# GoatWu/AdaLog

Hardware: NVIDIA B200
Metric: fpcs_candidates_per_s (higher is better)
Workload: dtype int8 + bf16 operands holding exact integers (s32 / f32 accumulate), f64 error sums

## Files before the change

### adalog_b200/_lib.py

```python
import ctypes
import os

_HERE = os.path.dirname(os.path.abspath(__file__))
LIB_PATH = os.path.join(_HERE, 'csrc', 'libadalog_b200.so')

c_f32p = ctypes.c_void_p
c_i64 = ctypes.c_int64
c_int = ctypes.c_int
c_vp = ctypes.c_void_p


class GemmErrArgs(ctypes.Structure):
    _fields_ = [
        ('A', c_vp), ('Bm', c_vp), ('a_rows', c_i64), ('b_rows', c_i64),
        ('KB', ctypes.c_int32), ('N', ctypes.c_int32), ('BN', ctypes.c_int32), ('U', ctypes.c_int32),
        ('UG', ctypes.c_int32), ('upc', ctypes.c_int32), ('S', ctypes.c_int32), ('dtype', ctypes.c_int32),
        ('order', ctypes.c_int32), ('reserved', ctypes.c_int32),
        ('brpg', c_i64), ('g_base', c_i64), ('u_base', c_i64),
        ('y', c_vp), ('ldy', c_i64),
        ('rs', c_vp), ('rb', c_vp), ('rs_div', c_i64), ('rs_mod', c_i64),
        ('cs', c_vp), ('cb', c_vp),
        ('partial', c_vp),
    ]

# ... 32 lines not shown
    'adalog_uniform_fakequant_f32': [c_vp, c_vp, c_vp, c_i64, c_vp, c_vp, c_i64, c_i64, c_int, c_int, c_vp],
    'adalog_log_fakequant_f32': [c_vp, c_vp, c_vp, c_i64, c_vp, c_int, c_int, c_vp, c_vp, c_vp, c_vp, c_int, c_vp],
    'adalog_twin_fakequant_f32': [c_vp, c_vp, c_i64, c_vp, c_int, c_vp],
    'adalog_sweep_err_w_self': [c_vp, c_int, c_int, c_vp, c_vp, c_int, c_int, c_vp, c_vp],
    'adalog_sweep_err_a_self': [c_vp, c_i64, c_int, c_int, c_vp, c_vp, c_int, c_int, c_vp, c_int, c_vp],
    'adalog_gen_uniform_fixed': [c_vp, c_i64, c_int, c_i64, c_vp, c_vp, c_i64, c_i64, c_int, c_vp, c_int, c_vp, c_int, c_vp],
    'adalog_gen_uniform_cand': [c_vp, c_i64, c_int, c_i64, c_vp, c_vp, c_int, c_i64, c_i64, c_i64, c_i64, c_i64, c_int,
                                c_vp, c_int, c_int, c_vp, c_int, c_vp],
    'adalog_gen_log_cand': [c_vp, c_i64, c_int, c_i64, c_vp, c_vp, c_int, c_vp, c_vp, c_int, c_vp, c_int, c_vp],
    'adalog_gen_log_fixed': [c_vp, c_i64, c_int, c_i64, c_vp, c_vp, c_vp, c_vp, c_vp, c_int, c_vp, c_int, c_vp],
    'adalog_gen_split3': [c_vp, c_i64, c_int, c_i64, c_vp, c_int, c_vp],
    'adalog_select_init': [c_vp, c_i64, c_int, c_vp, c_vp],
    'adalog_select_hist': [c_vp, c_i64, c_i64, c_i64, c_vp, c_i64, c_i64, c_int, c_int, c_int, c_vp],
    'adalog_select_scan': [c_vp, c_i64, c_int, c_int, c_vp],
    'adalog_select_finish': [c_vp, c_i64, c_int, c_vp, c_vp],
    'adalog_cand_gemm_err_grid': [ctypes.POINTER(GemmErrArgs)],
    'adalog_cand_gemm_err': [ctypes.POINTER(GemmErrArgs), c_vp],
    'adalog_fused_cand_gemm_err_grid': [ctypes.POINTER(FusedArgs)],
    'adalog_fused_cand_gemm_err': [ctypes.POINTER(FusedArgs), c_vp],
    'adalog_lin_fused_cand_gemm_err_grid': [ctypes.POINTER(LinFusedArgs)],
    'adalog_lin_fused_cand_gemm_err_passes': [ctypes.POINTER(LinFusedArgs)],
    'adalog_lin_fused_cand_gemm_err': [ctypes.POINTER(LinFusedArgs), c_vp],
    'adalog_gemm_dequant': [ctypes.POINTER(GemmErrArgs), c_vp, c_i64, c_i64, c_vp],
    'adalog_debug_gemm_tile': [c_vp, c_vp, c_int, c_int, c_vp, c_vp, c_vp, c_vp, c_int, c_vp],
}

OTHER_SYMBOLS = {'adalog_last_error', 'adalog_select_workspace_bytes', 'adalog_select_hist_ptr'}

_lib = None
LAUNCHES = {'count': 0}
_NO_LAUNCH = {'adalog_version', 'adalog_cand_gemm_err_grid', 'adalog_fused_cand_gemm_err_grid',
              'adalog_lin_fused_cand_gemm_err_grid', 'adalog_lin_fused_cand_gemm_err_passes'}


class AdalogError(RuntimeError):
    pass


def load():
    global _lib
    if _lib is not None:
        return _lib
    if not os.path.exists(LIB_PATH):
        raise AdalogError(f'{LIB_PATH} not found: build it with `python __graft_entry__.py` '
                          f'(adalog_b200 has no CPU fallback)')
    lib = ctypes.CDLL(LIB_PATH)
# ... 23 lines not shown
```

### adalog_b200/csrc/gemm_err.cu

```cuda
#include "common.cuh"
#include "tc_common.cuh"
#include "../../include/adalog_b200.h"
#include <cuda.h>
#include <cudaTypedefs.h>
#include <stdlib.h>
#include <type_traits>

namespace adalog {

constexpr int kMaxBN = 256;
constexpr int kStages = 4;
constexpr int kAccStages = 2;
constexpr uint32_t kABytes = kBM * kBK * 2;
constexpr uint32_t kBBytes = kMaxBN * kBK * 2;
constexpr uint32_t kTmemCols = 512;
constexpr int kEpiWarp0 = 0;
constexpr int kEpiWarps = 8;
constexpr int kEpiGroups = kEpiWarps / 4;
constexpr int kEpiThreads = kEpiWarps * 32;
constexpr int kTmaWarp = kEpiWarps, kMmaWarp = kEpiWarps + 1;
constexpr int kThreads = (kMmaWarp + 1) * 32;

constexpr int kCsCols = 1024;
constexpr int kSlabsPerGroup = (kMaxBN / 32 + kEpiGroups - 1) / kEpiGroups;
struct __align__(16) SmemTail {
  float ysw[kEpiWarps][kSlabsPerGroup * 32];
  float cs_all[kCsCols + kMaxBN];
  float cb_all[kCsCols + kMaxBN];
  uint64_t full[kStages];
  uint64_t empty[kStages];
  uint64_t tfull[kAccStages];
  uint64_t tempty[kAccStages];
  uint32_t tmem_base;
  uint32_t pad;
  double comb[kEpiGroups - 1][kBM];
};
constexpr size_t kSmemBytes = 1024  + (size_t)kStages * (kABytes + kBBytes);

struct KArgs {
  int KB, N, BN, NT, U, UG, upc, cpg;
  int gx, S, split_fast;
  long long brpg, g_base, u_base;
  const float* y; long long ldy;
  const float* rs; const float* rb; long long rs_div, rs_mod;
  const float* cs; const float* cb;
  double* partial;
  float* dbg;
  float* out; long long ldo; long long m_rows;
};

enum { MODE_CS = 0, MODE_RB = 1, MODE_PLAIN = 2, MODE_NOEPI = 3 ,
       MODE_STORE = 4 };

template <int MODE, bool DEBUG, bool I8>
__global__ void __maxnreg__(152)
cand_gemm_err_kernel(const __grid_constant__ CUtensorMap tmA, const __grid_constant__ CUtensorMap tmB, const KArgs a) {
  extern __shared__ uint8_t smem_raw[];
  uint8_t* smem = reinterpret_cast<uint8_t*>((reinterpret_cast<uintptr_t>(smem_raw) + 1023) & ~(uintptr_t)1023);
  uint8_t* sA = smem;
  uint8_t* sB = smem + (size_t)kStages * kABytes;
  __shared__ SmemTail tail_s;
  SmemTail* tail = &tail_s;

  const int warp = uniform_warp_idx();
  const int lane = threadIdx.x & 31;

  const int bx = a.split_fast ? (int)(blockIdx.x / a.S) : (int)(blockIdx.x % a.gx);
  const int by = a.split_fast ? (int)(blockIdx.x % a.S) : (int)(blockIdx.x / a.gx);
  const int g_local = bx / a.cpg;
  const int ci = bx - g_local * a.cpg;
  const int u0 = g_local * a.UG + (int)(((long long)ci * a.UG) / a.cpg);
  const int u1 = min(g_local * a.UG + (int)(((long long)(ci + 1) * a.UG) / a.cpg), a.U);
  const int nt0 = (int)(((long long)by * a.NT) / a.S);
  const int nt1 = (int)(((long long)(by + 1) * a.NT) / a.S);
  const int n_units = max(u1 - u0, 0);
// ... 38 lines not shown
    }
  } else if (warp == kMmaWarp) {
    {
      uint32_t stage = 0, phase = 0;
      const uint32_t idesc = I8 ? make_idesc_i8(a.BN) : make_idesc(a.BN);
      const uint32_t sA_u = smem_u32(sA), sB_u = smem_u32(sB);
      for (int t = 0; t < n_tiles; ++t) {
        const uint32_t as = t & 1, aphase = (t >> 1) & 1;
        mbar_wait(&tail->tempty[as], aphase ^ 1);
        tc_fence_after();
        const uint32_t tmem_d = tmem_base + as * kMaxBN;
        for (int kb = 0; kb < a.KB; ++kb) {
          mbar_wait(&tail->full[stage], phase);
          tc_fence_after();
          umma_kblock_commit<I8>(tmem_d, make_smem_desc(sA_u + stage * kABytes), make_smem_desc(sB_u + stage * kBBytes),
                                 idesc, kb != 0 ? 1u : 0u, 4, smem_u32(&tail->empty[stage]));
          if (++stage == kStages) { stage = 0; phase ^= 1; }
        }
        umma_commit_elect(smem_u32(&tail->tfull[as]));
      }
    }
  } else if (warp < kTmaWarp) {
    constexpr bool HAS_CS = MODE == MODE_CS || MODE == MODE_STORE;
    constexpr bool STORE = MODE == MODE_STORE;
    const int ew = warp - kEpiWarp0;
    const int eg = ew >> 2;
    const int et = ((warp & 3) << 5) | lane;
    const uint32_t lane_base = (uint32_t)((warp & 3) * 32) << 16;
    constexpr int G = kEpiGroups;
    float* const ysw = tail_s.ysw[ew];
    TwoSumF acc;
    float rs = 0.0f, rb = 0.0f;
    long long cur_ri = -1;
    float yreg[kSlabsPerGroup];
#pragma unroll
    for (int i = 0; i < kSlabsPerGroup; ++i) yreg[i] = 0.0f;
    if (HAS_CS) {
      const int st = threadIdx.x - kEpiWarp0 * 32;
      const int ncs = n_nt * a.BN;
      for (int idx = st; idx < kCsCols + kMaxBN; idx += kEpiThreads) {
        float cv = 0.0f, bv = 0.0f;
        if (idx < ncs) {
          const int ti = idx / a.BN;
          const int c = idx - ti * a.BN;
          const int n = (nt0 + ti) * a.BN + c;
          if (n < a.N) { cv = __ldg(a.cs + n); bv = __ldg(a.cb + n); }
        }
        tail_s.cs_all[idx] = cv;
        tail_s.cb_all[idx] = bv;
      }
      asm volatile("bar.sync 1, %0;" ::"n"(kEpiThreads) : "memory");
    }
    auto prefetch = [&](int u, int n0) {
#pragma unroll
      for (int i = 0; i < kSlabsPerGroup; ++i) {
        const int c = (eg + i * G) * 32 + lane;
        const int n = n0 + c;
        yreg[i] = (!STORE && c < a.BN && n < a.N) ? __ldg(a.y + (long long)u * a.ldy + n) : 0.0f;
      }
    };
    float acc4[4];
    auto accf = [](uint32_t w) -> float { return I8 ? __int2float_rn((int)w) : __uint_as_float(w); };
    float* orow = nullptr;
    int ocol = 0;
    const bool ovec = STORE && (a.ldo & 3) == 0 && (reinterpret_cast<uintptr_t>(a.out) & 15) == 0;
    auto quad = [&](auto masked, const uint32_t (&d)[32], int j, int l0, int cc, int lim, float rs, float rb) {
      constexpr bool MASKED = decltype(masked)::value;
      const float4 yv = *reinterpret_cast<const float4*>(&ysw[l0 + j]);
      const float y4[4] = {yv.x, yv.y, yv.z, yv.w};
      float c4[4] = {1.0f, 1.0f, 1.0f, 1.0f};
      if (HAS_CS) {
        const float4 cv = *reinterpret_cast<const float4*>(&tail_s.cs_all[cc + j]);
        c4[0] = cv.x; c4[1] = cv.y; c4[2] = cv.z; c4[3] = cv.w;
      }
      if (STORE) {
        const float4 bv = *reinterpret_cast<const float4*>(&tail_s.cb_all[cc + j]);
        float4 o;
        o.x = fmaf(rs * c4[0], accf(d[j + 0]), bv.x); o.y = fmaf(rs * c4[1], accf(d[j + 1]), bv.y);
        o.z = fmaf(rs * c4[2], accf(d[j + 2]), bv.z); o.w = fmaf(rs * c4[3], accf(d[j + 3]), bv.w);
        if (orow != nullptr) {
          float* dst = orow + ocol + j;
          if (!MASKED || j + 3 < lim) {
            if (ovec) *reinterpret_cast<float4*>(dst) = o;
            else { dst[0] = o.x; dst[1] = o.y; dst[2] = o.z; dst[3] = o.w; }
          } else {
            if (j + 0 < lim) dst[0] = o.x;
            if (j + 1 < lim) dst[1] = o.y;
            if (j + 2 < lim) dst[2] = o.z;
          }
        }
        return;
      }
      if (!MASKED) {
        const float f0 = accf(d[j]), f1 = accf(d[j + 1]), f2 = accf(d[j + 2]), f3 = accf(d[j + 3]);
        float e0, e1, e2, e3;
        if (HAS_CS) {
          float t0, t1, t2, t3;
          fmul2(t0, t1, f0, f1, c4[0], c4[1]);
          fmul2(t2, t3, f2, f3, c4[2], c4[3]);
          ffma2(e0, e1, -rs, -rs, t0, t1, y4[0], y4[1]);
          ffma2(e2, e3, -rs, -rs, t2, t3, y4[2], y4[3]);
        } else if (MODE == MODE_RB) {
// ... 7 lines not shown
          ffma2(e2, e3, -rs, -rs, f2, f3, y4[2], y4[3]);
        }
        ffma2(acc4[0], acc4[1], e0, e1, e0, e1, acc4[0], acc4[1]);
        ffma2(acc4[2], acc4[3], e2, e3, e2, e3, acc4[2], acc4[3]);
        return;
      }
#pragma unroll
      for (int e = 0; e < 4; ++e) {
        float diff;
        if (HAS_CS) diff = fmaf(-rs, accf(d[j + e]) * c4[e], y4[e]);
        else if (MODE == MODE_RB) diff = y4[e] - fmaf(rs, accf(d[j + e]), rb);
        else diff = fmaf(-rs, accf(d[j + e]), y4[e]);
        diff = (j + e < lim) ? diff : 0.0f;
        acc4[e] = fmaf(diff, diff, acc4[e]);
      }
    };
    auto consume = [&](const uint32_t (&d)[32], int c0, int l0, int cc, int lim, float rs, float rb, int n0, int ncols) {
      if (DEBUG) {
#pragma unroll
        for (int j = 0; j < 32; ++j)
          if (c0 + j < ncols) a.dbg[(long long)et * a.N + n0 + c0 + j] = accf(d[j]);
      }
      ocol = c0;
      if (MODE == MODE_NOEPI) {
        acc4[0] += __uint_as_float(d[0]);
      } else if (lim >= 32) {
#pragma unroll
        for (int j = 0; j < 32; j += 4) quad(std::false_type{}, d, j, l0, cc, 32, rs, rb);
      } else {
#pragma unroll
        for (int j = 0; j < 32; j += 4)
          if (j < lim) quad(std::true_type{}, d, j, l0, cc, lim, rs, rb);
      }
    };
    int cu = u0, cnt = 0;
    long long ri = 0, rrem = 0;
    if (n_tiles > 0) {
      const long long gu = a.u_base + cu;
      ri = (gu / a.rs_div) % a.rs_mod;
      rrem = gu % a.rs_div;
      prefetch(cu, (nt0 + cnt) * a.BN);
    }
    for (int t = 0; t < n_tiles; ++t) {
      const int n0 = (nt0 + cnt) * a.BN;
      const int toff = cnt * a.BN;
      const int ncols = min(a.BN, a.N - n0);
      const long long ri_t = ri;
      if (STORE) {
        const long long row = (a.u_base + cu) * kBM + et;
        orow = row < a.m_rows ? a.out + row * a.ldo + n0 : nullptr;
      }
      if (++cnt == n_nt) {
        cnt = 0; ++cu;
        if (++rrem == a.rs_div) { rrem = 0; if (++ri == a.rs_mod) ri = 0; }
      }
      const uint32_t as = t & 1, aphase = (t >> 1) & 1;
      __syncwarp();
#pragma unroll
      for (int i = 0; i < kSlabsPerGroup; ++i)
        ysw[i * 32 + lane] = HAS_CS ? yreg[i] - tail_s.cb_all[toff + (eg + i * G) * 32 + lane] : yreg[i];
      __syncwarp();
      if (t + 1 < n_tiles) prefetch(cu, (nt0 + cnt) * a.BN);
      if (ri_t != cur_ri) {
        cur_ri = ri_t;
        rs = __ldg(a.rs + ri_t * kBM + et);
        rb = (MODE == MODE_RB) ? __ldg(a.rb + ri_t * kBM + et) : 0.0f;
      }
      mbar_wait(&tail->tfull[as], aphase);
      tc_fence_after();
      acc4[0] = acc4[1] = acc4[2] = acc4[3] = 0.0f;
      const uint32_t tbase = tmem_base + lane_base + as * kMaxBN;
      const int nslab = (ncols + 31) >> 5;
      uint32_t da[32], db[32];
      if (eg < nslab) tmem_ld32(tbase + eg * 32, da);
      int l0 = 0;
      constexpr bool SLAB64 = MODE == MODE_RB;
      auto flush = [&]() {
        acc.add((acc4[0] + acc4[1]) + (acc4[2] + acc4[3]));
        acc4[0] = acc4[1] = acc4[2] = acc4[3] = 0.0f;
      };
      for (int sl = eg; sl < nslab; sl += 2 * G, l0 += 64) {
        tmem_ld_wait();
        if (sl + G < nslab) tmem_ld32(tbase + (sl + G) * 32, db);
        consume(da, sl * 32, l0, toff + sl * 32, ncols - sl * 32, rs, rb, n0, ncols);
        if (SLAB64) flush();
        if (sl + G < nslab) {
          tmem_ld_wait();
          if (sl + 2 * G < nslab) tmem_ld32(tbase + (sl + 2 * G) * 32, da);
          consume(db, (sl + G) * 32, l0 + 32, toff + (sl + G) * 32, ncols - (sl + G) * 32, rs, rb, n0, ncols);
          if (SLAB64) flush();
        }
      }
      if (!SLAB64) acc.add((acc4[0] + acc4[1]) + (acc4[2] + acc4[3]));
      tc_fence_before();
      __syncwarp();
      if (lane == 0) mbar_arrive(&tail->tempty[as]);
    }
    const double acc64 = acc.value();
    if (eg > 0) tail_s.comb[eg - 1][et] = acc64;
    asm volatile("bar.sync 1, %0;" ::"n"(kEpiThreads) : "memory");
    if (eg == 0 && a.partial) {
      double tot = acc64;
#pragma unroll
      for (int g = 1; g < kEpiGroups; ++g) tot += tail_s.comb[g - 1][et];
      a.partial[((long long)by * a.gx + bx) * kBM + et] = tot;
    }
  }

  tc_fence_before();
  __syncthreads();
  if (warp == kMmaWarp) {
    __syncwarp();
    tc_fence_after();
    asm volatile("tcgen05.dealloc.cta_group::1.sync.aligned.b32 %0, %1;" ::"r"(tmem_base), "r"(kTmemCols) : "memory");
  }
}

static int validate(const adalog_gemm_err_args* a, bool need_partial) {
  ADALOG_REQUIRE(a && a->A && a->Bm, -1, "cand_gemm_err: null operand");
  ADALOG_REQUIRE(a->KB > 0 && a->N > 0 && a->U > 0 && a->UG > 0 && a->upc > 0 && a->S > 0, -1,
                 "cand_gemm_err: non-positive size");
  ADALOG_REQUIRE(a->BN >= 16 && a->BN <= kMaxBN && a->BN % 16 == 0, -1, "cand_gemm_err: BN must be a multiple of 16 in [16,256]");
  ADALOG_REQUIRE(a->dtype == ADALOG_BF16 || a->dtype == ADALOG_I8, -1, "cand_gemm_err: dtype must be ADALOG_BF16 or ADALOG_I8");
  ADALOG_REQUIRE(a->order == ADALOG_ORDER_UNIT_FAST || a->order == ADALOG_ORDER_SPLIT_FAST, -1, "cand_gemm_err: bad order");
  ADALOG_REQUIRE(a->U % a->UG == 0, -1, "cand_gemm_err: U must be a multiple of UG");
  ADALOG_REQUIRE(a->a_rows >= (int64_t)a->U * kBM, -1, "cand_gemm_err: A has fewer than U*128 rows");
  ADALOG_REQUIRE(a->rs_div > 0 && a->rs_mod > 0 && a->rs, -1, "cand_gemm_err: row scale required");
  ADALOG_REQUIRE((a->cs == nullptr) == (a->cb == nullptr), -1, "cand_gemm_err: cs and cb come together");
  ADALOG_REQUIRE(!a->rb || a->cs || a->BN % 32 == 0, -1,
                 "cand_gemm_err: with a row bias (W-side sweeps) BN must be a multiple of 32 (per-slab FP64 promotion)");
  ADALOG_REQUIRE(a->y && (a->partial || !need_partial), -1, "cand_gemm_err: y / partial required");
  const int NT = (a->N + a->BN - 1) / a->BN;
  ADALOG_REQUIRE(a->S <= NT, -1, "cand_gemm_err: more N splits than N tiles");
  ADALOG_REQUIRE(!a->cs || ((NT + a->S - 1) / a->S) * a->BN <= kCsCols, -1,
                 "cand_gemm_err: with column scales a CTA covers at most 1024 columns (raise S)");
  return 0;
}

static int launch(const adalog_gemm_err_args* a, float* dbg, cudaStream_t st, float* out = nullptr, long long ldo = 0,
                  long long m_rows = 0) {
  KArgs k;
  k.out = out; k.ldo = ldo; k.m_rows = m_rows;
  k.KB = a->KB; k.N = a->N; k.BN = a->BN; k.NT = (a->N + a->BN - 1) / a->BN; k.U = a->U; k.UG = a->UG; k.upc = a->upc;
  k.cpg = (a->UG + a->upc - 1) / a->upc;
  k.brpg = a->brpg; k.g_base = a->g_base; k.u_base = a->u_base;
  k.y = a->y; k.ldy = a->ldy; k.rs = a->rs; k.rb = a->rb; k.rs_div = a->rs_div; k.rs_mod = a->rs_mod;
  k.cs = a->cs; k.cb = a->cb; k.partial = a->partial; k.dbg = dbg;
  CUtensorMap tmA, tmB;
  const bool i8 = a->dtype == ADALOG_I8;
  const int64_t cols = (int64_t)a->KB * (i8 ? 2 * kBK : kBK);
  int rc = make_map(&tmA, a->A, a->a_rows, cols, kBM, i8);
  if (rc) return rc;
  rc = make_map(&tmB, a->Bm, a->b_rows, cols, a->BN, i8);
  if (rc) return rc;
  k.gx = (a->U / a->UG) * k.cpg; k.S = a->S; k.split_fast = a->order == ADALOG_ORDER_SPLIT_FAST;
  dim3 grid((unsigned)((long long)k.gx * k.S));
#define ADALOG_LAUNCH_GEMM(MD, DBG, I8)                                                                       \
  do {                                                                                                        \
    cudaFuncSetAttribute(cand_gemm_err_kernel<MD, DBG, I8>, cudaFuncAttributeMaxDynamicSharedMemorySize,      \
                         (int)kSmemBytes);                                                                    \
    cand_gemm_err_kernel<MD, DBG, I8><<<grid, kThreads, kSmemBytes, st>>>(tmA, tmB, k);                       \
  } while (0)
  if (out) {
    if (i8) ADALOG_LAUNCH_GEMM(MODE_STORE, false, true);
    else    ADALOG_LAUNCH_GEMM(MODE_STORE, false, false);
  } else if (i8) {
    if (dbg)         ADALOG_LAUNCH_GEMM(MODE_PLAIN, true, true);
    else if (a->cs)  ADALOG_LAUNCH_GEMM(MODE_CS, false, true);
    else if (a->rb)  ADALOG_LAUNCH_GEMM(MODE_RB, false, true);
    else             ADALOG_LAUNCH_GEMM(MODE_PLAIN, false, true);
  } else {
    if (dbg)         ADALOG_LAUNCH_GEMM(MODE_PLAIN, true, false);
    else if (a->cs)  ADALOG_LAUNCH_GEMM(MODE_CS, false, false);
    else if (a->rb)  ADALOG_LAUNCH_GEMM(MODE_RB, false, false);
    else if (getenv("ADALOG_B200_DIAG_NOEPI")) ADALOG_LAUNCH_GEMM(MODE_NOEPI, false, false);
    else             ADALOG_LAUNCH_GEMM(MODE_PLAIN, false, false);
  }
#undef ADALOG_LAUNCH_GEMM
  return check_launch("cand_gemm_err");
}

}

using namespace adalog;

extern "C" {
// ... 1 lines not shown
int adalog_cand_gemm_err_grid(const adalog_gemm_err_args* a) {
  int rc = validate(a, false);
  if (rc) return rc;
  return (a->U / a->UG) * ((a->UG + a->upc - 1) / a->upc);
}

int adalog_cand_gemm_err(const adalog_gemm_err_args* a, void* stream) {
  int rc = validate(a, true);
  if (rc) return rc;
  return launch(a, nullptr, (cudaStream_t)stream);
}

int adalog_gemm_dequant(const adalog_gemm_err_args* a, float* out, int64_t ldo, int64_t m_rows, void* stream) {
  ADALOG_REQUIRE(a && out && m_rows > 0 && ldo >= a->N, -1, "gemm_dequant: bad output");
  ADALOG_REQUIRE(a->A && a->Bm && a->rs && a->cs && a->cb && a->KB > 0 && a->N > 0 && a->U > 0 && a->UG == a->U &&
                     a->upc > 0 && a->S > 0 && (int64_t)a->U * kBM >= m_rows && a->rs_div > 0 && a->rs_mod > 0, -1,
                 "gemm_dequant: bad arguments (one group, U = ceil(m_rows / 128), rs / cs / cb required)");
  ADALOG_REQUIRE(a->BN >= 16 && a->BN <= kMaxBN && a->BN % 16 == 0, -1, "gemm_dequant: BN must be a multiple of 16 in [16,256]");
  ADALOG_REQUIRE(a->dtype == ADALOG_BF16 || a->dtype == ADALOG_I8, -1, "gemm_dequant: dtype");
  ADALOG_REQUIRE(a->order == ADALOG_ORDER_UNIT_FAST || a->order == ADALOG_ORDER_SPLIT_FAST, -1, "gemm_dequant: order");
  const int NT = (a->N + a->BN - 1) / a->BN;
  ADALOG_REQUIRE(a->S <= NT && ((NT + a->S - 1) / a->S) * a->BN <= kCsCols, -1,
                 "gemm_dequant: a CTA covers at most 1024 columns (raise S)");
  return launch(a, nullptr, (cudaStream_t)stream, out, ldo, m_rows);
}

int adalog_debug_gemm_tile(const void* A, const void* Bm, int KB, int N, float* D, const float* zeros, const float* ones,
                           double* partial, int dtype, void* stream) {
  ADALOG_REQUIRE(A && Bm && D && zeros && ones && partial && KB > 0 && N > 0, -1, "debug_gemm_tile: bad arguments");
  double* part = partial;
  adalog_gemm_err_args a;
  memset(&a, 0, sizeof(a));
  a.A = A; a.Bm = Bm; a.a_rows = kBM; a.b_rows = N; a.KB = KB; a.N = N; a.dtype = dtype;
  a.BN = N >= kMaxBN ? kMaxBN : ((N + 15) / 16) * 16;
  a.U = 1; a.UG = 1; a.upc = 1; a.S = 1; a.brpg = N; a.g_base = 0; a.u_base = 0;
  a.y = zeros; a.ldy = 0; a.rs = ones; a.rb = nullptr; a.rs_div = 1; a.rs_mod = 1; a.cs = nullptr; a.cb = nullptr;
  a.partial = part;
  int rc = validate(&a, true);
  if (rc) return rc;
  return launch(&a, D, (cudaStream_t)stream);
}

}
```

### adalog_b200/ops.py

```python
import ctypes
import math
import threading

import torch

from . import _lib
from ._lib import AdalogError, FusedArgs, GemmErrArgs, LinFusedArgs
from ._lib import call as _lib_call

P_TILE = 128
BK = 64

PROFILE = {'on': False, 'gemm': [], 'fused': [], 'lin': []}


def profile_reset(on):
    PROFILE['on'] = bool(on)
    PROFILE['gemm'] = []
    PROFILE['fused'] = []
    PROFILE['lin'] = []


def profile_gemm_summary(split=False):
    torch.cuda.synchronize()
# ... 286 lines not shown
    else:
        call('adalog_cand_gemm_err', ctypes.byref(a), _stream())
    return partial


def gemm_dequant(A, m_rows, Bm, ka, N, rs, cs, cb, upc, S, i8=False, split_fast=False, out=None):
    _cuda(A, Bm, rs, cs, cb)
    BN = pick_bn(N)
    U = (m_rows + P_TILE - 1) // P_TILE
    a = GemmErrArgs()
    a.A, a.Bm = A.data_ptr(), Bm.data_ptr()
    a.a_rows, a.b_rows = int(m_rows), int(Bm.shape[0])
    a.KB = ka // (2 * BK if i8 else BK)
    a.dtype = I8 if i8 else BF16
    a.order = 1 if split_fast else 0
    a.N, a.BN, a.U, a.UG, a.upc, a.S = int(N), int(BN), int(U), int(U), int(upc), int(S)
    a.brpg, a.g_base, a.u_base = 0, 0, 0
    a.rs, a.rs_div, a.rs_mod = rs.data_ptr(), 1 << 62, 1
    a.cs, a.cb = cs.data_ptr(), cb.data_ptr()
    if out is None:
        out = torch.empty(m_rows, N, dtype=torch.float32, device=A.device)
    call('adalog_gemm_dequant', ctypes.byref(a), _p(out), int(out.stride(0)), int(m_rows), _stream())
    return out


SMEM_LIMIT = 227 * 1024 - 16384


def fused_plan(K, N, i8, log, n_levels):
    el = 2 * BK if i8 else BK
    KB = (K + el - 1) // el
    if N > 256 or KB > 4:
        return None
    BN = pick_bn(N)
    smem = 1024 + KB * 16384 + KB * BN * 128 + (P_TILE * (2 * n_levels + 1) * 4 if log else 0)
    if smem > SMEM_LIMIT or (log and (i8 or 2 * n_levels > 64)):
        return None
    return KB, BN


def fused_cand_gemm_err(x2d, K, Bm, N, U, UG, brpg, y, ldy, rs, rs_div, rs_mod, upc, n_levels, P, cs=None, cz=None,
                        pstride=0, gstride=0, g_div=1, g_mod=1, cq=None, mtab=None, i8=False):
    log = cq is not None
    KB, BN = fused_plan(K, N, i8, log, n_levels)
    _cuda(x2d, Bm, y, rs)
    assert x2d.dtype == torch.float32 and x2d.stride(1) == 1
# ... 102 lines not shown
```

### adalog_b200/sweep.py

```python
import functools
import math
import os

import torch

from . import _const, ops
from .quantizers._ste import flag as _flag
from .utils import dist as adist

WS_BYTES = int(os.environ.get('ADALOG_B200_WS_MB', '8192')) << 20
NUM_SMS = 148
R_BASE = 37.0
USE_I8 = os.environ.get('ADALOG_B200_I8', '1') == '1'

LIN_FUSED = os.environ.get('ADALOG_B200_LIN_FUSED', '1') != '0'


def _lin_fused_passes():
    mode = os.environ.get('ADALOG_B200_LIN_FUSED', '1')
    if not LIN_FUSED or mode == '0':
        return None
    return 1 << 30 if mode == 'force' else 1

_workspaces = {}
# ... 49 lines not shown
    if NT > 1 and unit_bytes * min(NUM_SMS, nu) > L2_CAND_BYTES:
        split_fast = True
        s_min = min(NT, max(s_min, math.ceil(unit_bytes * NUM_SMS / L2_CAND_TARGET)))
    best = None
    for S in range(s_min, min(NT, max(s_min, 16)) + 1):
        tps = math.ceil(NT / S)
        cands = {ug, 1}
        for w in range(1, 9):
            c = (NUM_SMS * w) // (groups * S)
            if c >= 1:
                cands.add(math.ceil(ug / min(c, ug)))
        for upc in cands:
            cpg = math.ceil(ug / upc)
            ctas = groups * cpg * S
            cost = math.ceil(ctas / NUM_SMS) * (math.ceil(ug / cpg) * tps * tile_cost + CTA_FIXED_COST)
            key = (cost, ctas)
            if best is None or key < best[0]:
                best = (key, upc, cpg, S)
    _, upc, cpg, S = best
    return groups, upc, cpg, S, split_fast


def run_cand_gemm(gen_cand, U, ka, UG, Bm, brpg, N, y, ldy, rs, rb=None, rs_div=1, rs_mod=1, cs=None, cb=None,
                  k_true=None, i8=False):
    dev = Bm.device
    single = UG == U
    unit_elems = ops.P_TILE * ka * (1 if i8 else 2)
    max_units = max(1, (WS_BYTES // 2) // unit_elems)
    step = min(U, max_units) if single else min(U, max(1, max_units // UG) * UG)
    n_chunks = (U + step - 1) // step
    BN = ops.pick_bn(N, 32 if rb is not None else 16)
    NT = (N + BN - 1) // BN
    overlap = OVERLAP and n_chunks > 1 and dev.type == 'cuda'
    ws_all = _workspace(dev, (2 if overlap else 1) * step * unit_elems)
    bufs = [ws_all[:step * unit_elems], ws_all[step * unit_elems:]] if overlap else [ws_all]

    def gemm(u0, nu, buf):
        ug = nu if single else UG
        groups, upc, cpg, S, sf = _launch_plan(nu, ug, NT, N * ka * (1 if i8 else 2), unit_elems,
                                               max((ka // 64) * BN * (1 if i8 else 2), 8 * BN),
                                               (1024 // BN) if cs is not None else 1 << 30)
        part = ops.cand_gemm_err(buf, nu * ops.P_TILE, Bm, ka, N, nu, ug, brpg, 0 if single else u0 // UG, u0, y,
                                 u0 * ldy, ldy, rs, rb, rs_div, rs_mod, cs, cb, upc, S, BN, k_true, i8, sf)
        return part.view(S, groups, cpg, ops.P_TILE).sum(dim=(0, 2))

    outs = []
    if not overlap:
        for u0 in range(0, U, step):
            nu = min(step, U - u0)
            gen_cand(u0, nu, bufs[0])
            outs.append(gemm(u0, nu, bufs[0]))
        return torch.cat(outs, dim=0)

    main = torch.cuda.current_stream(dev)
    s_gen, s_mma = _side_streams(dev)
    start = main.record_event()
    s_gen.wait_event(start)
    s_mma.wait_event(start)
    freed = [None, None]
    for i, u0 in enumerate(range(0, U, step)):
        nu = min(step, U - u0)
        b = i & 1
        with torch.cuda.stream(s_gen):
            if freed[b] is not None:
# ... 93 lines not shown
    with torch.no_grad():
        return ops.gen_split3(q(x2d))


def _fixed_act_operand(ctx, aq, i8=False):
    if _is_adalog(aq):
        def build_log():
            nl = aq.n_levels
            m2 = torch.round(_f32(aq.table2) * (4 * nl - 2))
            Bm = ops.gen_log_fixed(ctx.x2d, aq.scale, aq.q, aq.shift, aq.table1, m2, nl)
            return Bm, _f32(aq.scale).double().reshape(1) / (4 * nl - 2), _f32(aq.shift).double().reshape(1), 1
        return _cached_fixed(ctx, 'act', ('log', aq.n_levels) + _pkey(aq.scale, aq.q, aq.shift, aq.table1, aq.table2),
                             build_log)
    if getattr(aq, 'is_log', False) or type(aq).__name__ != 'UniformQuantizer':
        return _generic_fixed_operand(aq, ctx.x2d), torch.ones(1, dtype=torch.float64, device=ctx.x2d.device), None, 3

    def build_uniform():
        s, z = uniform_operand_params(aq)
        Bm, _ = ops.gen_uniform_fixed(ctx.x2d, s, z, 1 << 62, 1, aq.n_levels, i8=i8)
        return Bm, s.double(), None, 1
    return _cached_fixed(ctx, 'act', ('uniform', aq.n_levels, bool(i8)) + _pkey(aq.scale, aq.zero_point), build_uniform)


def linear_err_w(ctx, weight3, bias, aq, cs, cz, n_levels_w):
    n_V, rows, in_f = weight3.shape
    out_f = n_V * rows
    P = cs.shape[0]
    dev = weight3.device
    c2, z2 = _cand2d(cs, cz)
    i8 = type(aq).__name__ == 'UniformQuantizer' and _i8_ok(aq.n_levels, n_levels_w)
    Bm, a_scale, shift, krep = _fixed_act_operand(ctx, aq, i8)
    ka = krep * ops.kpad(in_f, i8)
    W2d = _f32(weight3).reshape(out_f, in_f)
    c2p = _pad128(c2.t().contiguous())
    rs = (c2p.double() * a_scale).float().contiguous()
    b = _f32(bias) if bias is not None else torch.zeros(out_f, device=dev)
    rb = b.reshape(-1, 1).expand(out_f, ops.P_TILE).contiguous()
    rowsum = torch.empty(out_f, ops.P_TILE, dtype=torch.float32, device=dev) if shift is not None else None

    def gen(u0, nu, out):
        ops.gen_uniform_cand(W2d, u0, nu, c2, z2, P, out_f, 1, 1, out_f, n_levels_w, out, krep,
                             rowsum[u0:] if rowsum is not None else None, i8=i8)
        if shift is not None:
            rb[u0:u0 + nu] = (b[u0:u0 + nu].double().reshape(-1, 1)
                              - shift * c2p[u0:u0 + nu].double() * rowsum[u0:u0 + nu].double()).float()

    ntok = ctx.x2d.shape[0]
    res = run_cand_gemm(gen, out_f, ka, 1, Bm, 0, ntok, ctx.yT, ntok, rs, rb, 1, out_f, k_true=in_f, i8=i8)
    res = adist.all_reduce_sum(res)
    sims = -(res[:, :P] / ctx.tok_per_sample)
    return sims.t().float().reshape(P, n_V, rows)


def _fixed_weight_operand(weight3, wq, i8=False, ctx=None):
# ... 332 lines not shown
```

### include/adalog_b200.h

```cpp
#ifndef ADALOG_B200_H_
#define ADALOG_B200_H_

#include <stdint.h>

#ifdef __cplusplus
extern "C" {
#endif

#define ADALOG_P 128
#define ADALOG_BK 64
#define ADALOG_BF16 0
#define ADALOG_I8 1
#define ADALOG_ORDER_UNIT_FAST 0
#define ADALOG_ORDER_SPLIT_FAST 1

int adalog_version(void);
const char* adalog_last_error(void);


int adalog_uniform_fakequant_f32(const float* x, float* y, int16_t* codes, int64_t n, const float* scale,
                                 const float* zp, int64_t inner, int64_t ngroups, int n_levels, int symmetric,
                                 void* stream);

int adalog_log_fakequant_f32(const float* x, float* y, int16_t* codes, int64_t n, const float* scale, int kind,
// ... 39 lines not shown
  const void* A;      const void* Bm;
  int64_t a_rows;     int64_t b_rows;
  int32_t KB;
  int32_t N;
  int32_t BN;
  int32_t U;
  int32_t UG;
  int32_t upc;
  int32_t S;
  int32_t dtype;
  int32_t order;
  int32_t reserved;
  int64_t brpg;
  int64_t g_base;     int64_t u_base;
  const float* y;     int64_t ldy;
  const float* rs;    const float* rb;  int64_t rs_div; int64_t rs_mod;
  const float* cs;    const float* cb;
  double* partial;
} adalog_gemm_err_args;

int adalog_cand_gemm_err_grid(const adalog_gemm_err_args* a);
int adalog_cand_gemm_err(const adalog_gemm_err_args* a, void* stream);

#define ADALOG_GEN_UNIFORM 0
#define ADALOG_GEN_LOG 1
typedef struct {
  const float* x;     int64_t ldx;
  const void* Bm;     int64_t b_rows;
  int32_t K;
  int32_t KB;
  int32_t N;
  int32_t BN;
  int32_t U;          int32_t UG;          int32_t upc;
  int32_t P;          int32_t n_levels;
  int32_t gen;        int32_t dtype;
  int32_t epi_warps;
  int64_t brpg;       int64_t g_base;      int64_t u_base;
  const float* cs;    const float* cz;     int64_t pstride; int64_t gstride; int64_t g_div; int64_t g_mod;
  const long long* cq; const float* mtab;
  const float* y;     int64_t ldy;
  const float* rs;    int64_t rs_div;      int64_t rs_mod;
  double* partial;
} adalog_fused_args;

int adalog_fused_cand_gemm_err_grid(const adalog_fused_args* a);
int adalog_fused_cand_gemm_err(const adalog_fused_args* a, void* stream);
// ... 28 lines not shown
```

Measured before the change: 73330.

## Score weight candidates via Gram-matrix quadratic form instead of per-token GEMM

For uniform int8 linear layers with many tokens, the squared output error of each weight candidate is expanded algebraically as rs²·wᵀGw − 2·rs·wᵀU + ‖y−b‖². G=AᵀA and U=Aᵀ(y−b) are precomputed once with exact int8 GEMMs, using digit-plane splitting of the fixed-point targets and of G. The candidate GEMM then runs against the Gram matrix with K×K cost instead of tokens×K, and a new epilogue mode reduces the exact integer quadratic form and the linear term per row. This removes the dependence of sweep cost on token count. In exchange it adds a precompute stage, fixed-point rounding of the targets, overflow bound checks that fall back to the old path, and the extra work of G's digit planes.

After: 77490, median of 6. +5.7%, better.

```diff
diff --git a/adalog_b200/_lib.py b/adalog_b200/_lib.py
--- a/adalog_b200/_lib.py
+++ b/adalog_b200/_lib.py
@@ -78,6 +78,8 @@
     'adalog_lin_fused_cand_gemm_err_passes': [ctypes.POINTER(LinFusedArgs)],
     'adalog_lin_fused_cand_gemm_err': [ctypes.POINTER(LinFusedArgs), c_vp],
     'adalog_gemm_dequant': [ctypes.POINTER(GemmErrArgs), c_vp, c_i64, c_i64, c_vp],
+    'adalog_gemm_i32': [ctypes.POINTER(GemmErrArgs), c_vp, c_i64, c_i64, c_vp],
+    'adalog_gram_qform': [ctypes.POINTER(GemmErrArgs), c_vp, c_vp, c_vp, c_vp],
     'adalog_debug_gemm_tile': [c_vp, c_vp, c_int, c_int, c_vp, c_vp, c_vp, c_vp, c_int, c_vp],
 }
 
diff --git a/adalog_b200/csrc/gemm_err.cu b/adalog_b200/csrc/gemm_err.cu
--- a/adalog_b200/csrc/gemm_err.cu
+++ b/adalog_b200/csrc/gemm_err.cu
@@ -34,6 +34,7 @@
   uint32_t tmem_base;
   uint32_t pad;
   double comb[kEpiGroups - 1][kBM];
+  double comb2[kEpiGroups - 1][kBM];
 };
 constexpr size_t kSmemBytes = 1024  + (size_t)kStages * (kABytes + kBBytes);
 
@@ -47,10 +48,11 @@
   double* partial;
   float* dbg;
   float* out; long long ldo; long long m_rows;
+  const int8_t* wc; int ka; const double* gu; long long* qpart; double* lpart;
 };
 
 enum { MODE_CS = 0, MODE_RB = 1, MODE_PLAIN = 2, MODE_NOEPI = 3 ,
-       MODE_STORE = 4 };
+       MODE_STORE = 4, MODE_RAW = 5, MODE_GRAM = 6 };
 
 template <int MODE, bool DEBUG, bool I8>
 __global__ void __maxnreg__(152)
@@ -135,7 +137,10 @@
     }
   } else if (warp < kTmaWarp) {
     constexpr bool HAS_CS = MODE == MODE_CS || MODE == MODE_STORE;
-    constexpr bool STORE = MODE == MODE_STORE;
+    constexpr bool STORE = MODE == MODE_STORE || MODE == MODE_RAW;
+    constexpr bool RAW = MODE == MODE_RAW;
+    constexpr bool GRAM = MODE == MODE_GRAM;
+    constexpr bool NEED_Y = !STORE && !GRAM;
     const int ew = warp - kEpiWarp0;
     const int eg = ew >> 2;
     const int et = ((warp & 3) << 5) | lane;
@@ -169,11 +174,14 @@
       for (int i = 0; i < kSlabsPerGroup; ++i) {
         const int c = (eg + i * G) * 32 + lane;
         const int n = n0 + c;
-        yreg[i] = (!STORE && c < a.BN && n < a.N) ? __ldg(a.y + (long long)u * a.ldy + n) : 0.0f;
+        yreg[i] = (NEED_Y && c < a.BN && n < a.N) ? __ldg(a.y + (long long)u * a.ldy + n) : 0.0f;
       }
     };
     float acc4[4];
     auto accf = [](uint32_t w) -> float { return I8 ? __int2float_rn((int)w) : __uint_as_float(w); };
+    unsigned long long gq = 0;
+    double gl = 0.0;
+    int cu_t = 0;
     float* orow = nullptr;
     int ocol = 0;
     const bool ovec = STORE && (a.ldo & 3) == 0 && (reinterpret_cast<uintptr_t>(a.out) & 15) == 0;
@@ -187,10 +195,15 @@
         c4[0] = cv.x; c4[1] = cv.y; c4[2] = cv.z; c4[3] = cv.w;
       }
       if (STORE) {
-        const float4 bv = *reinterpret_cast<const float4*>(&tail_s.cb_all[cc + j]);
         float4 o;
-        o.x = fmaf(rs * c4[0], accf(d[j + 0]), bv.x); o.y = fmaf(rs * c4[1], accf(d[j + 1]), bv.y);
-        o.z = fmaf(rs * c4[2], accf(d[j + 2]), bv.z); o.w = fmaf(rs * c4[3], accf(d[j + 3]), bv.w);
+        if (RAW) {
+          o.x = __uint_as_float(d[j + 0]); o.y = __uint_as_float(d[j + 1]);
+          o.z = __uint_as_float(d[j + 2]); o.w = __uint_as_float(d[j + 3]);
+        } else {
+          const float4 bv = *reinterpret_cast<const float4*>(&tail_s.cb_all[cc + j]);
+          o.x = fmaf(rs * c4[0], accf(d[j + 0]), bv.x); o.y = fmaf(rs * c4[1], accf(d[j + 1]), bv.y);
+          o.z = fmaf(rs * c4[2], accf(d[j + 2]), bv.z); o.w = fmaf(rs * c4[3], accf(d[j + 3]), bv.w);
+        }
         if (orow != nullptr) {
           float* dst = orow + ocol + j;
           if (!MASKED || j + 3 < lim) {
@@ -244,7 +257,30 @@
           if (c0 + j < ncols) a.dbg[(long long)et * a.N + n0 + c0 + j] = accf(d[j]);
       }
       ocol = c0;
-      if (MODE == MODE_NOEPI) {
+      if (GRAM) {
+        const int n = n0 + c0;
+        const int plane = n / a.ka;
+        const int kk = n - plane * a.ka;
+        const int8_t* wp = a.wc + ((long long)cu_t * kBM + et) * a.ka + kk;
+        const int4 w0 = __ldg(reinterpret_cast<const int4*>(wp));
+        const int4 w1 = __ldg(reinterpret_cast<const int4*>(wp + 16));
+        const int wv[8] = {w0.x, w0.y, w0.z, w0.w, w1.x, w1.y, w1.z, w1.w};
+        long long q = 0;
+#pragma unroll
+        for (int j = 0; j < 32; ++j) {
+          const int w = (int)((unsigned)wv[j >> 2] << (24 - 8 * (j & 3))) >> 24;
+          if (j < lim) q += (long long)(int)d[j] * w;
+        }
+        gq += (unsigned long long)q << (8 * plane);
+        if (plane == 0) {
+          const double* up = a.gu + (a.u_base + cu_t) * (long long)a.ka + kk;
+#pragma unroll
+          for (int j = 0; j < 32; ++j) {
+            const int w = (int)((unsigned)wv[j >> 2] << (24 - 8 * (j & 3))) >> 24;
+            if (j < lim) gl = fma((double)w, __ldg(up + j), gl);
+          }
+        }
+      } else if (MODE == MODE_NOEPI) {
         acc4[0] += __uint_as_float(d[0]);
       } else if (lim >= 32) {
 #pragma unroll
@@ -268,6 +304,7 @@
       const int toff = cnt * a.BN;
       const int ncols = min(a.BN, a.N - n0);
       const long long ri_t = ri;
+      cu_t = cu;
       if (STORE) {
         const long long row = (a.u_base + cu) * kBM + et;
         orow = row < a.m_rows ? a.out + row * a.ldo + n0 : nullptr;
@@ -283,7 +320,7 @@
         ysw[i * 32 + lane] = HAS_CS ? yreg[i] - tail_s.cb_all[toff + (eg + i * G) * 32 + lane] : yreg[i];
       __syncwarp();
       if (t + 1 < n_tiles) prefetch(cu, (nt0 + cnt) * a.BN);
-      if (ri_t != cur_ri) {
+      if (!RAW && !GRAM && ri_t != cur_ri) {
         cur_ri = ri_t;
         rs = __ldg(a.rs + ri_t * kBM + et);
         rb = (MODE == MODE_RB) ? __ldg(a.rb + ri_t * kBM + et) : 0.0f;
@@ -318,6 +355,22 @@
       __syncwarp();
       if (lane == 0) mbar_arrive(&tail->tempty[as]);
     }
+    if (GRAM) {
+      if (eg > 0) { tail_s.comb[eg - 1][et] = __longlong_as_double((long long)gq); tail_s.comb2[eg - 1][et] = gl; }
+      asm volatile("bar.sync 1, %0;" ::"n"(kEpiThreads) : "memory");
+      if (eg == 0) {
+        unsigned long long tq = gq;
+        double tl = gl;
+#pragma unroll
+        for (int g = 1; g < kEpiGroups; ++g) {
+          tq += (unsigned long long)__double_as_longlong(tail_s.comb[g - 1][et]);
+          tl += tail_s.comb2[g - 1][et];
+        }
+        const long long idx = ((long long)by * a.gx + bx) * kBM + et;
+        a.qpart[idx] = (long long)tq;
+        a.lpart[idx] = tl;
+      }
+    } else {
     const double acc64 = acc.value();
     if (eg > 0) tail_s.comb[eg - 1][et] = acc64;
     asm volatile("bar.sync 1, %0;" ::"n"(kEpiThreads) : "memory");
@@ -326,6 +379,7 @@
 #pragma unroll
       for (int g = 1; g < kEpiGroups; ++g) tot += tail_s.comb[g - 1][et];
       a.partial[((long long)by * a.gx + bx) * kBM + et] = tot;
+    }
     }
   }
 
@@ -359,10 +413,15 @@
   return 0;
 }
 
+enum { LAUNCH_ERR, LAUNCH_STORE, LAUNCH_RAW, LAUNCH_GRAM };
+
 static int launch(const adalog_gemm_err_args* a, float* dbg, cudaStream_t st, float* out = nullptr, long long ldo = 0,
-                  long long m_rows = 0) {
+                  long long m_rows = 0, int kind = LAUNCH_ERR, const double* gu = nullptr, long long* qpart = nullptr,
+                  double* lpart = nullptr) {
   KArgs k;
+  memset(&k, 0, sizeof(k));
   k.out = out; k.ldo = ldo; k.m_rows = m_rows;
+  k.wc = static_cast<const int8_t*>(a->A); k.ka = a->KB * 2 * kBK; k.gu = gu; k.qpart = qpart; k.lpart = lpart;
   k.KB = a->KB; k.N = a->N; k.BN = a->BN; k.NT = (a->N + a->BN - 1) / a->BN; k.U = a->U; k.UG = a->UG; k.upc = a->upc;
   k.cpg = (a->UG + a->upc - 1) / a->upc;
   k.brpg = a->brpg; k.g_base = a->g_base; k.u_base = a->u_base;
@@ -383,7 +442,11 @@
                          (int)kSmemBytes);                                                                    \
     cand_gemm_err_kernel<MD, DBG, I8><<<grid, kThreads, kSmemBytes, st>>>(tmA, tmB, k);                       \
   } while (0)
-  if (out) {
+  if (kind == LAUNCH_RAW) {
+    ADALOG_LAUNCH_GEMM(MODE_RAW, false, true);
+  } else if (kind == LAUNCH_GRAM) {
+    ADALOG_LAUNCH_GEMM(MODE_GRAM, false, true);
+  } else if (out) {
     if (i8) ADALOG_LAUNCH_GEMM(MODE_STORE, false, true);
     else    ADALOG_LAUNCH_GEMM(MODE_STORE, false, false);
   } else if (i8) {
@@ -431,7 +494,34 @@
   const int NT = (a->N + a->BN - 1) / a->BN;
   ADALOG_REQUIRE(a->S <= NT && ((NT + a->S - 1) / a->S) * a->BN <= kCsCols, -1,
                  "gemm_dequant: a CTA covers at most 1024 columns (raise S)");
-  return launch(a, nullptr, (cudaStream_t)stream, out, ldo, m_rows);
+  return launch(a, nullptr, (cudaStream_t)stream, out, ldo, m_rows, LAUNCH_STORE);
+}
+
+int adalog_gemm_i32(const adalog_gemm_err_args* a, int32_t* out, int64_t ldo, int64_t m_rows, void* stream) {
+  ADALOG_REQUIRE(a && out && m_rows > 0 && ldo >= a->N, -1, "gemm_i32: bad output");
+  ADALOG_REQUIRE(a->A && a->Bm && a->KB > 0 && a->N > 0 && a->U > 0 && a->UG == a->U && a->upc > 0 && a->S > 0 &&
+                     (int64_t)a->U * kBM >= m_rows && a->rs_div > 0 && a->rs_mod > 0, -1,
+                 "gemm_i32: bad arguments (one group, U = ceil(m_rows / 128))");
+  ADALOG_REQUIRE(a->BN >= 32 && a->BN <= kMaxBN && a->BN % 32 == 0, -1, "gemm_i32: BN must be a multiple of 32 in [32,256]");
+  ADALOG_REQUIRE(a->dtype == ADALOG_I8, -1, "gemm_i32: int8 operands only (S32 accumulation)");
+  ADALOG_REQUIRE(a->order == ADALOG_ORDER_UNIT_FAST || a->order == ADALOG_ORDER_SPLIT_FAST, -1, "gemm_i32: order");
+  ADALOG_REQUIRE(a->S <= (a->N + a->BN - 1) / a->BN, -1, "gemm_i32: more N splits than N tiles");
+  return launch(a, nullptr, (cudaStream_t)stream, reinterpret_cast<float*>(out), ldo, m_rows, LAUNCH_RAW);
+}
+
+int adalog_gram_qform(const adalog_gemm_err_args* a, const double* U, int64_t* qpartial, double* lpartial, void* stream) {
+  ADALOG_REQUIRE(a && a->A && a->Bm && U && qpartial && lpartial, -1, "gram_qform: null operand");
+  ADALOG_REQUIRE(a->KB > 0 && a->N > 0 && a->U > 0 && a->UG == 1 && a->upc > 0 && a->S > 0, -1,
+                 "gram_qform: bad sizes (one unit = one weight row per group)");
+  ADALOG_REQUIRE(a->dtype == ADALOG_I8, -1, "gram_qform: int8 operands only");
+  ADALOG_REQUIRE(a->BN >= 32 && a->BN <= kMaxBN && a->BN % 32 == 0, -1, "gram_qform: BN must be a multiple of 32 in [32,256]");
+  ADALOG_REQUIRE(a->N % (a->KB * 2 * kBK) == 0, -1, "gram_qform: N must be a whole number of digit planes of ka rows");
+  ADALOG_REQUIRE(a->order == ADALOG_ORDER_UNIT_FAST || a->order == ADALOG_ORDER_SPLIT_FAST, -1, "gram_qform: bad order");
+  ADALOG_REQUIRE(a->a_rows >= (int64_t)a->U * kBM && a->rs_div > 0 && a->rs_mod > 0, -1, "gram_qform: bad A / row maps");
+  ADALOG_REQUIRE(a->S <= (a->N + a->BN - 1) / a->BN, -1, "gram_qform: more N splits than N tiles");
+  ADALOG_REQUIRE((reinterpret_cast<uintptr_t>(a->A) & 15) == 0, -1, "gram_qform: A must be 16-byte aligned");
+  return launch(a, nullptr, (cudaStream_t)stream, nullptr, 0, 0, LAUNCH_GRAM, U, reinterpret_cast<long long*>(qpartial),
+                lpartial);
 }
 
 int adalog_debug_gemm_tile(const void* A, const void* Bm, int KB, int N, float* D, const float* zeros, const float* ones,
diff --git a/adalog_b200/ops.py b/adalog_b200/ops.py
--- a/adalog_b200/ops.py
+++ b/adalog_b200/ops.py
@@ -332,6 +332,51 @@
         out = torch.empty(m_rows, N, dtype=torch.float32, device=A.device)
     call('adalog_gemm_dequant', ctypes.byref(a), _p(out), int(out.stride(0)), int(m_rows), _stream())
     return out
+
+
+def _gemm_args(A, a_rows, Bm, ka, N, BN, U, UG, upc, S, split_fast):
+    a = GemmErrArgs()
+    a.A, a.Bm = A.data_ptr(), Bm.data_ptr()
+    a.a_rows, a.b_rows = int(a_rows), int(Bm.shape[0])
+    a.KB = ka // (2 * BK)
+    a.dtype = I8
+    a.order = 1 if split_fast else 0
+    a.N, a.BN, a.U, a.UG, a.upc, a.S = int(N), int(BN), int(U), int(UG), int(upc), int(S)
+    a.rs_div, a.rs_mod = 1 << 62, 1
+    return a
+
+
+def gemm_i32(A, m_rows, Bm, ka, N, upc, S, split_fast=False):
+    _cuda(A, Bm)
+    BN = pick_bn(N, 32)
+    U = (m_rows + P_TILE - 1) // P_TILE
+    a = _gemm_args(A, m_rows, Bm, ka, N, BN, U, U, upc, S, split_fast)
+    out = torch.empty(m_rows, N, dtype=torch.int32, device=A.device)
+    _timed('gemm', 2.0 * m_rows * N * ka, 'adalog_gemm_i32', ctypes.byref(a), _p(out), int(out.stride(0)), int(m_rows),
+           _stream())
+    return out
+
+
+def gram_qform(A, Bm, ka, N, U, u_base, Uf, upc, S, split_fast=False, BN=None):
+    _cuda(A, Bm, Uf)
+    BN = BN or pick_bn(N, 32)
+    a = _gemm_args(A, U * P_TILE, Bm, ka, N, BN, U, 1, upc, S, split_fast)
+    a.u_base = int(u_base)
+    q = torch.empty(S, U, P_TILE, dtype=torch.int64, device=A.device)
+    l = torch.empty(S, U, P_TILE, dtype=torch.float64, device=A.device)
+    _timed('gemm', 2.0 * P_TILE * U * N * ka, 'adalog_gram_qform', ctypes.byref(a), _p(Uf), _p(q), _p(l), _stream())
+    return q, l
+
+
+def _timed(kind, flops, name, *args):
+    if not PROFILE['on']:
+        return call(name, *args)
+    e0, e1 = torch.cuda.Event(enable_timing=True), torch.cuda.Event(enable_timing=True)
+    e0.record()
+    rc = call(name, *args)
+    e1.record()
+    PROFILE[kind].append((e0, e1, flops, True))
+    return rc
 
 
 SMEM_LIMIT = 227 * 1024 - 16384
diff --git a/adalog_b200/sweep.py b/adalog_b200/sweep.py
--- a/adalog_b200/sweep.py
+++ b/adalog_b200/sweep.py
@@ -95,14 +95,14 @@
 
 
 def run_cand_gemm(gen_cand, U, ka, UG, Bm, brpg, N, y, ldy, rs, rb=None, rs_div=1, rs_mod=1, cs=None, cb=None,
-                  k_true=None, i8=False):
+                  k_true=None, i8=False, gram=None):
     dev = Bm.device
     single = UG == U
     unit_elems = ops.P_TILE * ka * (1 if i8 else 2)
     max_units = max(1, (WS_BYTES // 2) // unit_elems)
     step = min(U, max_units) if single else min(U, max(1, max_units // UG) * UG)
     n_chunks = (U + step - 1) // step
-    BN = ops.pick_bn(N, 32 if rb is not None else 16)
+    BN = ops.pick_bn(N, 32 if rb is not None or gram is not None else 16)
     NT = (N + BN - 1) // BN
     overlap = OVERLAP and n_chunks > 1 and dev.type == 'cuda'
     ws_all = _workspace(dev, (2 if overlap else 1) * step * unit_elems)
@@ -113,6 +113,9 @@
         groups, upc, cpg, S, sf = _launch_plan(nu, ug, NT, N * ka * (1 if i8 else 2), unit_elems,
                                                max((ka // 64) * BN * (1 if i8 else 2), 8 * BN),
                                                (1024 // BN) if cs is not None else 1 << 30)
+        if gram is not None:
+            q, l = ops.gram_qform(buf, Bm, ka, N, nu, u0, gram, upc, S, sf, BN)
+            return torch.stack([q.sum(dim=0), l.sum(dim=0).view(torch.int64)], dim=1)
         part = ops.cand_gemm_err(buf, nu * ops.P_TILE, Bm, ka, N, nu, ug, brpg, 0 if single else u0 // UG, u0, y,
                                  u0 * ldy, ldy, rs, rb, rs_div, rs_mod, cs, cb, upc, S, BN, k_true, i8, sf)
         return part.view(S, groups, cpg, ops.P_TILE).sum(dim=(0, 2))
@@ -252,7 +255,142 @@
     return _cached_fixed(ctx, 'act', ('uniform', aq.n_levels, bool(i8)) + _pkey(aq.scale, aq.zero_point), build_uniform)
 
 
-def linear_err_w(ctx, weight3, bias, aq, cs, cz, n_levels_w):
+GRAM_F = 27
+GRAM_Y_MAX = 2.0 ** 9
+GRAM_Y_PLANES = 5
+GRAM_TOK_PER_K = 8
+_I63 = 1 << 62
+_TOK_CHUNK = 1 << 17
+
+
+def int8_digits(v, n):
+    out = []
+    for _ in range(n):
+        d = ((v + 128) & 255) - 128
+        out.append(d.to(torch.int8))
+        v = (v - d) >> 8
+    return torch.stack(out)
+
+
+def digit_planes(vmax):
+    n = 1
+    while vmax >= (1 << (8 * n - 1)) - (1 << (8 * (n - 1))):
+        n += 1
+    return n
+
+
+def combine_digits(parts):
+    acc = parts[-1].to(torch.int64)
+    for d in range(parts.shape[0] - 2, -1, -1):
+        acc = acc * 256 + parts[d].to(torch.int64)
+    return acc
+
+
+def gram_bounds_ok(tok_global, k_true, n_levels_w, g_max):
+    wmax = 2 * n_levels_w - 1
+    return 127 * (1 << 37) * tok_global <= _I63 and (wmax * k_true) ** 2 * g_max <= _I63
+
+
+def _tok_chunks(ntok):
+    return [(t0, min(ntok, t0 + _TOK_CHUNK)) for t0 in range(0, ntok, _TOK_CHUNK)]
+
+
+def _tok_major(m, t0, t1):
+    tp = ops.kpad(t1 - t0, True)
+    out = torch.zeros(m.shape[1], tp, dtype=torch.int8, device=m.device)
+    out[:, :t1 - t0] = m[t0:t1].t()
+    return out
+
+
+def _stats_gemm(A, B, ka_tok):
+    M, N = A.shape[0], B.shape[0]
+    U = (M + ops.P_TILE - 1) // ops.P_TILE
+    BN = ops.pick_bn(N, 32)
+    NT = (N + BN - 1) // BN
+    _, upc, _, S, sf = _launch_plan(U, U, NT, N * ka_tok, ops.P_TILE * ka_tok, max((ka_tok // 64) * BN, 8 * BN))
+    return ops.gemm_i32(A, M, B, ka_tok, N, upc, S, sf)
+
+
+def _gram_targets(ctx, bias, out_f):
+    def build():
+        y = ctx.y2d
+        ntok = y.shape[0]
+        scale = float(1 << GRAM_F)
+        b = _f32(bias) if bias is not None else torch.zeros(out_f, device=y.device)
+        b_fx = torch.round(b.double() * scale).long()
+        y_fx = torch.round(y.double() * scale).long()
+        d = y_fx - b_fx
+        h, l = d >> 19, d & ((1 << 19) - 1)
+        bad = (y.abs() > GRAM_Y_MAX).sum().reshape(1)
+        st = torch.cat([(h * h).sum(0), (h * l).sum(0), (l * l).sum(0), bad])
+        st = adist.all_reduce_sum(st)
+        if int(st[-1]) > 0 or float(b.abs().max()) > GRAM_Y_MAX:
+            return None
+        s2 = st[:3 * out_f].view(3, out_f).double()
+        S = (s2[0] * float(1 << 38) + s2[1] * float(1 << 20)) + s2[2]
+        planes = int8_digits(y_fx, GRAM_Y_PLANES)
+        del y_fx, d, h, l
+        ypl = [_tok_major(planes.permute(1, 0, 2).reshape(ntok, -1), t0, t1) for t0, t1 in _tok_chunks(ntok)]
+        return ypl, b_fx, S
+    return _cached_fixed(ctx, 'gram_y', _pkey(bias), build)
+
+
+def _gram_round(ctx, aq, bias, Bm, tgt, out_f, in_f, n_levels_w):
+    ypl, b_fx, S = tgt
+
+    def build():
+        ntok, ka = Bm.shape
+        G = torch.zeros(ka, ka, dtype=torch.int64, device=Bm.device)
+        UY = torch.zeros(ka, GRAM_Y_PLANES * out_f, dtype=torch.int64, device=Bm.device)
+        for (t0, t1), yc in zip(_tok_chunks(ntok), ypl):
+            At = _tok_major(Bm, t0, t1)
+            G += _stats_gemm(At, At, At.shape[1])
+            UY += _stats_gemm(At, yc, At.shape[1])
+        abar = Bm.sum(dim=0, dtype=torch.int64)
+        st = adist.all_reduce_sum(torch.cat([G.reshape(-1), UY.reshape(-1), abar]))
+        n_g, n_uy = ka * ka, UY.numel()
+        G = st[:n_g].view(ka, ka)
+        UY = combine_digits(st[n_g:n_g + n_uy].view(ka, GRAM_Y_PLANES, out_f).transpose(0, 1))
+        abar = st[n_g + n_uy:]
+        g_max = int(G.abs().max())
+        if not gram_bounds_ok(ntok * adist.world_size(), in_f, n_levels_w, g_max):
+            return None
+        U = UY - abar.view(ka, 1) * b_fx.view(1, out_f)
+        pg = digit_planes(g_max)
+        Gp = int8_digits(G, pg).reshape(pg * ka, ka).contiguous()
+        return Gp, U.t().double().contiguous()
+    return _cached_fixed(ctx, 'gram_a', ('uniform', aq.n_levels, n_levels_w) + _pkey(aq.scale, aq.zero_point, bias),
+                         build)
+
+
+def _linear_err_w_gram(ctx, weight3, bias, aq, cs, cz, n_levels_w, Bm, a_scale):
+    n_V, rows, in_f = weight3.shape
+    out_f = n_V * rows
+    P = cs.shape[0]
+    tgt = _gram_targets(ctx, bias, out_f)
+    if tgt is None:
+        return None
+    rnd = _gram_round(ctx, aq, bias, Bm, tgt, out_f, in_f, n_levels_w)
+    if rnd is None:
+        return None
+    Gp, Uf = rnd
+    S = tgt[2]
+    ka = Bm.shape[1]
+    c2, z2 = _cand2d(cs, cz)
+    W2d = _f32(weight3).reshape(out_f, in_f)
+
+    def gen(u0, nu, out):
+        ops.gen_uniform_cand(W2d, u0, nu, c2, z2, P, out_f, 1, 1, out_f, n_levels_w, out, i8=True)
+
+    res = run_cand_gemm(gen, out_f, ka, 1, Gp, 0, Gp.shape[0], None, 0, None, i8=True, gram=Uf)
+    Q, L = res[:, 0].double(), res[:, 1].view(torch.float64)
+    rs = _pad128(c2.t().contiguous()).double() * a_scale
+    E = (rs * rs * Q - (2.0 / (1 << GRAM_F)) * rs * L) + S.view(-1, 1) / float(1 << (2 * GRAM_F))
+    sims = -(E[:, :P] / ctx.tok_per_sample)
+    return sims.t().float().reshape(P, n_V, rows)
+
+
+def linear_err_w(ctx, weight3, bias, aq, cs, cz, n_levels_w, gram=None):
     n_V, rows, in_f = weight3.shape
     out_f = n_V * rows
     P = cs.shape[0]
@@ -260,6 +398,11 @@
     c2, z2 = _cand2d(cs, cz)
     i8 = type(aq).__name__ == 'UniformQuantizer' and _i8_ok(aq.n_levels, n_levels_w)
     Bm, a_scale, shift, krep = _fixed_act_operand(ctx, aq, i8)
+    if i8 and gram is not False and aq.scale.numel() == 1 and (
+            gram or ctx.x2d.shape[0] >= GRAM_TOK_PER_K * ops.kpad(in_f, True)):
+        sims = _linear_err_w_gram(ctx, weight3, bias, aq, cs, cz, n_levels_w, Bm, a_scale)
+        if sims is not None:
+            return sims
     ka = krep * ops.kpad(in_f, i8)
     W2d = _f32(weight3).reshape(out_f, in_f)
     c2p = _pad128(c2.t().contiguous())
diff --git a/include/adalog_b200.h b/include/adalog_b200.h
--- a/include/adalog_b200.h
+++ b/include/adalog_b200.h
@@ -85,6 +85,9 @@
 int adalog_cand_gemm_err_grid(const adalog_gemm_err_args* a);
 int adalog_cand_gemm_err(const adalog_gemm_err_args* a, void* stream);
 
+int adalog_gemm_i32(const adalog_gemm_err_args* a, int32_t* out, int64_t ldo, int64_t m_rows, void* stream);
+int adalog_gram_qform(const adalog_gemm_err_args* a, const double* U, int64_t* qpartial, double* lpartial, void* stream);
+
 #define ADALOG_GEN_UNIFORM 0
 #define ADALOG_GEN_LOG 1
 typedef struct {
```
